# xuelunshen/gim

Hardware: AMD Instinct MI355X
Metric: image-pairs/sec at 640x480 (higher is better)
Workload: dtype fp16

## Files before the change

### gim_amd/csrc/emit.hip

```cpp
#include "gim_common.h"

namespace {

struct Segs { gim_copy_segs s; };

__global__ void __launch_bounds__(256) copy_segments_kernel(const Segs a) {
    const int k = blockIdx.y;
    const char* src = (const char*)a.s.src[k];
    char* dst = (char*)a.s.dst[k];
    const int64_t n = a.s.bytes[k];
    const int64_t t = (int64_t)blockIdx.x * blockDim.x + threadIdx.x, nt = (int64_t)gridDim.x * blockDim.x;
    const bool vec = (((uintptr_t)src | (uintptr_t)dst) & 15) == 0;
    const int64_t nv = vec ? n >> 4 : 0;
    for (int64_t i = t; i < nv; i += nt) ((uint4*)dst)[i] = src ? ((const uint4*)src)[i] : make_uint4(0u, 0u, 0u, 0u);
    for (int64_t i = (nv << 4) + t; i < n; i += nt) dst[i] = src ? src[i] : (char)0;
}

__global__ void __launch_bounds__(256) pack_matches_kernel(const int64_t* __restrict__ m_bids, const float2* __restrict__ mk0,
                                                           const float2* __restrict__ mk1, const float* __restrict__ conf,
                                                           const int64_t* __restrict__ pair_ids, int64_t pid_base,
                                                           float* __restrict__ out, int M) {
    const int m = blockIdx.x * blockDim.x + threadIdx.x;
    if (m >= M) return;
    const int64_t b = m_bids[m];
    const float pid = (float)(pair_ids ? pair_ids[b] : pid_base + b);
    const float2 p0 = mk0[m], p1 = mk1[m];
    float* o = out + (size_t)m * 6;
    *(float2*)(o + 0) = make_float2(pid, p0.x);
    *(float2*)(o + 2) = make_float2(p0.y, p1.x);
    *(float2*)(o + 4) = make_float2(p1.y, conf[m]);
}

constexpr int TL_THREADS = 1024, TL_MAX_FLAGS = 32768;

template <bool REACH2, bool QUARTER>
__device__ __forceinline__ void fine_tile_list_body(const int64_t* __restrict__ b_ids, const int64_t* __restrict__ i_ids,
                                                    const int64_t* __restrict__ j_ids, const int* __restrict__ count, int cap,
                                                    int bs, int w0c, int w1c, int stride, int H, int W,
                                                    int* __restrict__ tiles, int* __restrict__ n_tiles, int tiles_cap,
                                                    int* __restrict__ tiles2, int* __restrict__ n_tiles2,
                                                    int* __restrict__ tilesq, int* __restrict__ n_tilesq, int tilesq_cap) {
    static_assert(!QUARTER || REACH2, "the quarter-level lists are derived from the +-4 flags");
    __shared__ __attribute__((aligned(16))) unsigned char flags[TL_MAX_FLAGS];
    __shared__ int part[TL_THREADS];
    __shared__ int part2[REACH2 ? TL_THREADS : 1];
    __shared__ int partq[QUARTER ? TL_THREADS : 1][2];
    const int t = threadIdx.x;
    const int tiles_x = (W + 31) / 32, tiles_y = (H + 7) / 8, per_img = tiles_x * tiles_y, nflags = 2 * bs * per_img;
    const int h = H / 2, w = W / 2, qtiles_x = w / 32, qtiles_y = h / 8, qper_img = qtiles_x * qtiles_y;
    const int qbase = (nflags + 3) & ~3, nqflags = QUARTER ? 2 * bs * qper_img : 0;
    for (int i = t; i < (QUARTER ? qbase + nqflags : nflags); i += TL_THREADS) flags[i] = 0;
    __syncthreads();
    int M = count[0];
    M = M < 0 ? 0 : (M < cap ? M : cap);
    for (int m = t; m < M; m += TL_THREADS) {
        const int64_t b = b_ids[m];
        if (b < 0 || b >= bs) continue;
#pragma unroll
        for (int side = 0; side < 2; ++side) {
            const int64_t cell = side ? j_ids[m] : i_ids[m];
            const int wc = side ? w1c : w0c;
            if (cell < 0 || cell >= (int64_t)wc * ((H + stride - 1) / stride)) continue;
            const int cy = (int)cell / wc, cx = (int)cell - cy * wc;
            int y0 = cy * stride - 3, y1 = cy * stride + 3, x0 = cx * stride - 3, x1 = cx * stride + 3;
            y0 = y0 < 0 ? 0 : y0; x0 = x0 < 0 ? 0 : x0;
            y1 = y1 > H - 1 ? H - 1 : y1; x1 = x1 > W - 1 ? W - 1 : x1;
            if (y0 > y1 || x0 > x1) continue;
            const int img = side * bs + (int)b;
            if constexpr (REACH2) {
                int Y0 = cy * stride - 4, Y1 = cy * stride + 4, X0 = cx * stride - 4, X1 = cx * stride + 4;
                Y0 = Y0 < 0 ? 0 : Y0; X0 = X0 < 0 ? 0 : X0;
                Y1 = Y1 > H - 1 ? H - 1 : Y1; X1 = X1 > W - 1 ? W - 1 : X1;
                for (int ty = Y0 >> 3; ty <= (Y1 >> 3); ++ty)
                    for (int tx = X0 >> 5; tx <= (X1 >> 5); ++tx) {
                        const bool in3 = ty >= (y0 >> 3) && ty <= (y1 >> 3) && tx >= (x0 >> 5) && tx <= (x1 >> 5);
                        const int f = (img * tiles_y + ty) * tiles_x + tx;
                        atomicOr((unsigned*)flags + (f >> 2), (in3 ? 3u : 2u) << (8 * (f & 3)));
                    }
            } else {
            for (int ty = y0 >> 3; ty <= (y1 >> 3); ++ty)
                for (int tx = x0 >> 5; tx <= (x1 >> 5); ++tx) flags[(img * tiles_y + ty) * tiles_x + tx] = 1;
            }
        }
    }
    __syncthreads();
    if constexpr (QUARTER) {
        unsigned char* const qf = flags + qbase;
        const float sy = (float)(h - 1) / (float)(H - 1), sx = (float)(w - 1) / (float)(W - 1);
        for (int i = t; i < nflags; i += TL_THREADS) {
            if (!(flags[i] & 2)) continue;
            const int img = i / per_img, r = i - img * per_img, ty = r / tiles_x, tx = r - ty * tiles_x;
            const int xa = (int)(sx * (32 * tx));
            const int xe = xa + 23 < w - 1 ? xa + 23 : w - 1;
            for (int Y = 8 * ty; Y < 8 * ty + 8 && Y < H; ++Y) {
                const float fy = sy * Y;
                const int y0 = (int)fy, y1 = y0 + (y0 < h - 1 ? 1 : 0);
#pragma unroll
                for (int d = 0; d < 3; ++d) {
                    const int ra = y0 - d > 0 ? y0 - d : 0, rb = y1 + d < h - 1 ? y1 + d : h - 1;
                    const int ca = xa - d > 0 ? xa - d : 0, cb = xe + d < w - 1 ? xe + d : w - 1;
                    const unsigned bits = d == 0 ? 7u : (d == 1 ? 6u : 4u);
                    for (int qy = ra >> 3; qy <= (rb >> 3); ++qy)
                        for (int qx = ca >> 5; qx <= (cb >> 5); ++qx) {
                            const int f = (img * qtiles_y + qy) * qtiles_x + qx;
                            if ((qf[f] & bits) != bits) atomicOr((unsigned*)qf + (f >> 2), bits << (8 * (f & 3)));
                        }
                }
            }
        }
        __syncthreads();
    }
    const int per = (nflags + TL_THREADS - 1) / TL_THREADS;
    const int lo = t * per < nflags ? t * per : nflags, hi = lo + per < nflags ? lo + per : nflags;
    int n = 0, n2 = 0;
    for (int i = lo; i < hi; ++i) { n += flags[i] & 1; n2 += flags[i] >> 1; }
    part[t] = n;
    if constexpr (REACH2) part2[t] = n2;
    const int qper = (nqflags + TL_THREADS - 1) / TL_THREADS;
    const int qlo = t * qper < nqflags ? t * qper : nqflags, qhi = qlo + qper < nqflags ? qlo + qper : nqflags;
    int nab = 0, nc = 0;
    if constexpr (QUARTER) {
        for (int i = qlo; i < qhi; ++i) {
            const int f = flags[qbase + i];
            nab += ((f >> 2) & 1) << 16 | ((f >> 1) & 1);
            nc += f & 1;
        }
        partq[t][0] = nab; partq[t][1] = nc;
    }
    __syncthreads();
    for (int d = 1; d < TL_THREADS; d <<= 1) {
        const int v = t >= d ? part[t - d] : 0;
        const int v2 = REACH2 && t >= d ? part2[t - d] : 0;
        const int vab = QUARTER && t >= d ? partq[t - d][0] : 0, vc = QUARTER && t >= d ? partq[t - d][1] : 0;
        __syncthreads();
        part[t] += v;
        if constexpr (REACH2) part2[t] += v2;
        if constexpr (QUARTER) { partq[t][0] += vab; partq[t][1] += vc; }
        __syncthreads();
    }
    int o = part[t] - n;
    for (int i = lo; i < hi; ++i)
        if (flags[i] & 1) {
            if (o < tiles_cap) tiles[o] = i;
            ++o;
        }
    if (t == TL_THREADS - 1) n_tiles[0] = part[t] < tiles_cap ? part[t] : tiles_cap;
    if constexpr (REACH2) {
        int o2 = part2[t] - n2;
        for (int i = lo; i < hi; ++i)
            if (flags[i] & 2) {
                if (o2 < tiles_cap) tiles2[o2] = i;
                ++o2;
            }
        if (t == TL_THREADS - 1) n_tiles2[0] = part2[t] < tiles_cap ? part2[t] : tiles_cap;
    }
    if constexpr (QUARTER) {
        int oa = (partq[t][0] >> 16) - (nab >> 16), ob = (partq[t][0] & 0xffff) - (nab & 0xffff), oc = partq[t][1] - nc;
        for (int i = qlo; i < qhi; ++i) {
            const int f = flags[qbase + i];
            if (f & 4) { if (oa < tilesq_cap) tilesq[oa] = i; ++oa; }
            if (f & 2) { if (ob < tilesq_cap) tilesq[tilesq_cap + ob] = i; ++ob; }
            if (f & 1) { if (oc < tilesq_cap) tilesq[2 * tilesq_cap + oc] = i; ++oc; }
        }
        if (t == TL_THREADS - 1) {
            const int ta = partq[t][0] >> 16, tb = partq[t][0] & 0xffff, tc = partq[t][1];
            n_tilesq[0] = ta < tilesq_cap ? ta : tilesq_cap;
            n_tilesq[1] = tb < tilesq_cap ? tb : tilesq_cap;
            n_tilesq[2] = tc < tilesq_cap ? tc : tilesq_cap;
        }
    }
}

template <bool REACH2>
__global__ void __launch_bounds__(TL_THREADS) fine_tile_list_kernel(const int64_t* __restrict__ b_ids, const int64_t* __restrict__ i_ids,
                                                                  const int64_t* __restrict__ j_ids, const int* __restrict__ count, int cap,
                                                                  int bs, int w0c, int w1c, int stride, int H, int W,
                                                                  int* __restrict__ tiles, int* __restrict__ n_tiles, int tiles_cap,
                                                                  int* __restrict__ tiles2, int* __restrict__ n_tiles2) {
    fine_tile_list_body<REACH2, false>(b_ids, i_ids, j_ids, count, cap, bs, w0c, w1c, stride, H, W, tiles, n_tiles, tiles_cap, tiles2, n_tiles2,
                                       nullptr, nullptr, 0);
}

__global__ void __launch_bounds__(TL_THREADS) fine_tile_lists4_kernel(const int64_t* __restrict__ b_ids, const int64_t* __restrict__ i_ids,
                                                                    const int64_t* __restrict__ j_ids, const int* __restrict__ count, int cap,
                                                                    int bs, int w0c, int w1c, int stride, int H, int W,
                                                                    int* __restrict__ tiles, int* __restrict__ n_tiles, int tiles_cap,
                                                                    int* __restrict__ tiles2, int* __restrict__ n_tiles2,
                                                                    int* __restrict__ tilesq, int* __restrict__ n_tilesq, int tilesq_cap) {
    fine_tile_list_body<true, true>(b_ids, i_ids, j_ids, count, cap, bs, w0c, w1c, stride, H, W, tiles, n_tiles, tiles_cap, tiles2, n_tiles2,
                                    tilesq, n_tilesq, tilesq_cap);
}

}

extern "C" int gim_fine_tile_list_max_flags(void) { return TL_MAX_FLAGS; }

extern "C" int gim_fine_tile_list(const int64_t* b_ids, const int64_t* i_ids, const int64_t* j_ids, const int* count, int cap, int bs,
                                  int w0c, int w1c, int stride, int H, int W, int* tiles, int* n_tiles, int tiles_cap, gim_stream_t stream) {
    GIM_REQUIRE(b_ids && i_ids && j_ids && count && tiles && n_tiles, "gim_fine_tile_list: NULL pointer");
    GIM_REQUIRE(cap >= 0 && bs > 0 && w0c > 0 && w1c > 0 && stride > 0 && H > 0 && W > 0, "gim_fine_tile_list: bad geometry");
    const int64_t nflags = 2ll * bs * ((W + 31) / 32) * ((H + 7) / 8);
    GIM_REQUIRE(nflags <= TL_MAX_FLAGS, "gim_fine_tile_list: %lld patches exceed the %d flags of the one-workgroup kernel", (long long)nflags, TL_MAX_FLAGS);
    GIM_REQUIRE(tiles_cap >= nflags, "gim_fine_tile_list: the list holds %d entries, the maps have %lld patches", tiles_cap, (long long)nflags);
    hipLaunchKernelGGL(fine_tile_list_kernel<false>, dim3(1), dim3(TL_THREADS), 0, (hipStream_t)stream, b_ids, i_ids, j_ids, count, cap, bs, w0c, w1c,
                       stride, H, W, tiles, n_tiles, tiles_cap, nullptr, nullptr);
    return gim_check_launch("fine_tile_list_kernel");
}

extern "C" int gim_fine_tile_lists(const int64_t* b_ids, const int64_t* i_ids, const int64_t* j_ids, const int* count, int cap, int bs,
                                   int w0c, int w1c, int stride, int H, int W, int* tiles, int* n_tiles, int* tiles4, int* n_tiles4,
                                   int tiles_cap, gim_stream_t stream) {
    GIM_REQUIRE(b_ids && i_ids && j_ids && count && tiles && n_tiles && tiles4 && n_tiles4, "gim_fine_tile_lists: NULL pointer");
    GIM_REQUIRE(cap >= 0 && bs > 0 && w0c > 0 && w1c > 0 && stride > 0 && H > 0 && W > 0, "gim_fine_tile_lists: bad geometry");
    const int64_t nflags = 2ll * bs * ((W + 31) / 32) * ((H + 7) / 8);
    GIM_REQUIRE(nflags <= TL_MAX_FLAGS, "gim_fine_tile_lists: %lld patches exceed the %d flags of the one-workgroup kernel", (long long)nflags, TL_MAX_FLAGS);
    GIM_REQUIRE(tiles_cap >= nflags, "gim_fine_tile_lists: the lists hold %d entries each, the maps have %lld patches", tiles_cap, (long long)nflags);
    hipLaunchKernelGGL(fine_tile_list_kernel<true>, dim3(1), dim3(TL_THREADS), 0, (hipStream_t)stream, b_ids, i_ids, j_ids, count, cap, bs, w0c, w1c,
                       stride, H, W, tiles, n_tiles, tiles_cap, tiles4, n_tiles4);
    return gim_check_launch("fine_tile_list_kernel");
}

extern "C" int gim_fine_tile_lists4(const int64_t* b_ids, const int64_t* i_ids, const int64_t* j_ids, const int* count, int cap, int bs,
                                    int w0c, int w1c, int stride, int H, int W, int* tiles, int* n_tiles, int* tiles4, int* n_tiles4,
                                    int tiles_cap, int* tilesq, int* n_tilesq, int tilesq_cap, gim_stream_t stream) {
    GIM_REQUIRE(b_ids && i_ids && j_ids && count && tiles && n_tiles && tiles4 && n_tiles4 && tilesq && n_tilesq, "gim_fine_tile_lists4: NULL pointer");
    GIM_REQUIRE(cap >= 0 && bs > 0 && w0c > 0 && w1c > 0 && stride > 0 && H > 0 && W > 0, "gim_fine_tile_lists4: bad geometry");
    GIM_REQUIRE(H % 16 == 0 && W % 64 == 0, "gim_fine_tile_lists4: the 1/4-resolution maps (%d x %d) must be whole 8 x 32 patches", H / 2, W / 2);
    const int64_t nflags = 2ll * bs * (W / 32) * (H / 8), nq = 2ll * bs * (W / 64) * (H / 16);
    GIM_REQUIRE(((nflags + 3) & ~3ll) + nq <= TL_MAX_FLAGS, "gim_fine_tile_lists4: %lld + %lld patches exceed the %d flags of the one-workgroup kernel",
                (long long)nflags, (long long)nq, TL_MAX_FLAGS);
    GIM_REQUIRE(tiles_cap >= nflags && tilesq_cap >= nq, "gim_fine_tile_lists4: the lists hold %d / %d entries each, the maps have %lld / %lld patches",
                tiles_cap, tilesq_cap, (long long)nflags, (long long)nq);
    hipLaunchKernelGGL(fine_tile_lists4_kernel, dim3(1), dim3(TL_THREADS), 0, (hipStream_t)stream, b_ids, i_ids, j_ids, count, cap, bs, w0c, w1c,
                       stride, H, W, tiles, n_tiles, tiles_cap, tiles4, n_tiles4, tilesq, n_tilesq, tilesq_cap);
    return gim_check_launch("fine_tile_lists4_kernel");
}

extern "C" int gim_copy_segments(const gim_copy_segs* sp, gim_stream_t stream) {
    GIM_REQUIRE(sp, "gim_copy_segments: NULL args");
    GIM_REQUIRE(sp->n >= 0 && sp->n <= GIM_MAX_COPY_SEGS, "gim_copy_segments: n=%d outside [0, %d]", sp->n, GIM_MAX_COPY_SEGS);
    int64_t mx = 0;
    for (int k = 0; k < sp->n; ++k) {
        GIM_REQUIRE(sp->bytes[k] >= 0 && (sp->bytes[k] == 0 || sp->dst[k]), "gim_copy_segments: segment %d: bad size / NULL dst", k);
        mx = sp->bytes[k] > mx ? sp->bytes[k] : mx;
    }
    if (sp->n == 0 || mx == 0) return GIM_OK;
    Segs a;
    a.s = *sp;
    int64_t blocks = (mx / 16 + 255) / 256;
    blocks = blocks < 1 ? 1 : (blocks > 1024 ? 1024 : blocks);
    hipLaunchKernelGGL(copy_segments_kernel, dim3((unsigned)blocks, (unsigned)sp->n), dim3(256), 0, (hipStream_t)stream, a);
    return gim_check_launch("copy_segments_kernel");
}

extern "C" int gim_pack_matches(const int64_t* m_bids, const float* mkpts0, const float* mkpts1, const float* mconf,
                                const int64_t* pair_ids, int64_t pid_base, float* out, int M, gim_stream_t stream) {
    GIM_REQUIRE(M >= 0, "gim_pack_matches: M=%d", M);
    if (M == 0) return GIM_OK;
    GIM_REQUIRE(m_bids && mkpts0 && mkpts1 && mconf && out, "gim_pack_matches: NULL pointer");
    hipLaunchKernelGGL(pack_matches_kernel, dim3((unsigned)((M + 255) / 256)), dim3(256), 0, (hipStream_t)stream, m_bids,
                       (const float2*)mkpts0, (const float2*)mkpts1, mconf, pair_ids, pid_base, out, M);
    return gim_check_launch("pack_matches_kernel");
}
```

Before: 970.8.

## Rewrite four-list tile kernel with wave-shuffle scans, prefetch and word-wide popcounts

```diff
diff --git a/gim_amd/csrc/emit.hip b/gim_amd/csrc/emit.hip
--- a/gim_amd/csrc/emit.hip
+++ b/gim_amd/csrc/emit.hip
@@ -33,23 +33,18 @@
 
 constexpr int TL_THREADS = 1024, TL_MAX_FLAGS = 32768;
 
-template <bool REACH2, bool QUARTER>
+template <bool REACH2>
 __device__ __forceinline__ void fine_tile_list_body(const int64_t* __restrict__ b_ids, const int64_t* __restrict__ i_ids,
                                                     const int64_t* __restrict__ j_ids, const int* __restrict__ count, int cap,
                                                     int bs, int w0c, int w1c, int stride, int H, int W,
                                                     int* __restrict__ tiles, int* __restrict__ n_tiles, int tiles_cap,
-                                                    int* __restrict__ tiles2, int* __restrict__ n_tiles2,
-                                                    int* __restrict__ tilesq, int* __restrict__ n_tilesq, int tilesq_cap) {
-    static_assert(!QUARTER || REACH2, "the quarter-level lists are derived from the +-4 flags");
+                                                    int* __restrict__ tiles2, int* __restrict__ n_tiles2) {
     __shared__ __attribute__((aligned(16))) unsigned char flags[TL_MAX_FLAGS];
     __shared__ int part[TL_THREADS];
     __shared__ int part2[REACH2 ? TL_THREADS : 1];
-    __shared__ int partq[QUARTER ? TL_THREADS : 1][2];
     const int t = threadIdx.x;
     const int tiles_x = (W + 31) / 32, tiles_y = (H + 7) / 8, per_img = tiles_x * tiles_y, nflags = 2 * bs * per_img;
-    const int h = H / 2, w = W / 2, qtiles_x = w / 32, qtiles_y = h / 8, qper_img = qtiles_x * qtiles_y;
-    const int qbase = (nflags + 3) & ~3, nqflags = QUARTER ? 2 * bs * qper_img : 0;
-    for (int i = t; i < (QUARTER ? qbase + nqflags : nflags); i += TL_THREADS) flags[i] = 0;
+    for (int i = t; i < nflags; i += TL_THREADS) flags[i] = 0;
     __syncthreads();
     int M = count[0];
     M = M < 0 ? 0 : (M < cap ? M : cap);
@@ -84,58 +79,19 @@
         }
     }
     __syncthreads();
-    if constexpr (QUARTER) {
-        unsigned char* const qf = flags + qbase;
-        const float sy = (float)(h - 1) / (float)(H - 1), sx = (float)(w - 1) / (float)(W - 1);
-        for (int i = t; i < nflags; i += TL_THREADS) {
-            if (!(flags[i] & 2)) continue;
-            const int img = i / per_img, r = i - img * per_img, ty = r / tiles_x, tx = r - ty * tiles_x;
-            const int xa = (int)(sx * (32 * tx));
-            const int xe = xa + 23 < w - 1 ? xa + 23 : w - 1;
-            for (int Y = 8 * ty; Y < 8 * ty + 8 && Y < H; ++Y) {
-                const float fy = sy * Y;
-                const int y0 = (int)fy, y1 = y0 + (y0 < h - 1 ? 1 : 0);
-#pragma unroll
-                for (int d = 0; d < 3; ++d) {
-                    const int ra = y0 - d > 0 ? y0 - d : 0, rb = y1 + d < h - 1 ? y1 + d : h - 1;
-                    const int ca = xa - d > 0 ? xa - d : 0, cb = xe + d < w - 1 ? xe + d : w - 1;
-                    const unsigned bits = d == 0 ? 7u : (d == 1 ? 6u : 4u);
-                    for (int qy = ra >> 3; qy <= (rb >> 3); ++qy)
-                        for (int qx = ca >> 5; qx <= (cb >> 5); ++qx) {
-                            const int f = (img * qtiles_y + qy) * qtiles_x + qx;
-                            if ((qf[f] & bits) != bits) atomicOr((unsigned*)qf + (f >> 2), bits << (8 * (f & 3)));
-                        }
-                }
-            }
-        }
-        __syncthreads();
-    }
     const int per = (nflags + TL_THREADS - 1) / TL_THREADS;
     const int lo = t * per < nflags ? t * per : nflags, hi = lo + per < nflags ? lo + per : nflags;
     int n = 0, n2 = 0;
     for (int i = lo; i < hi; ++i) { n += flags[i] & 1; n2 += flags[i] >> 1; }
     part[t] = n;
     if constexpr (REACH2) part2[t] = n2;
-    const int qper = (nqflags + TL_THREADS - 1) / TL_THREADS;
-    const int qlo = t * qper < nqflags ? t * qper : nqflags, qhi = qlo + qper < nqflags ? qlo + qper : nqflags;
-    int nab = 0, nc = 0;
-    if constexpr (QUARTER) {
-        for (int i = qlo; i < qhi; ++i) {
-            const int f = flags[qbase + i];
-            nab += ((f >> 2) & 1) << 16 | ((f >> 1) & 1);
-            nc += f & 1;
-        }
-        partq[t][0] = nab; partq[t][1] = nc;
-    }
     __syncthreads();
     for (int d = 1; d < TL_THREADS; d <<= 1) {
         const int v = t >= d ? part[t - d] : 0;
         const int v2 = REACH2 && t >= d ? part2[t - d] : 0;
-        const int vab = QUARTER && t >= d ? partq[t - d][0] : 0, vc = QUARTER && t >= d ? partq[t - d][1] : 0;
         __syncthreads();
         part[t] += v;
         if constexpr (REACH2) part2[t] += v2;
-        if constexpr (QUARTER) { partq[t][0] += vab; partq[t][1] += vc; }
         __syncthreads();
     }
     int o = part[t] - n;
@@ -154,20 +110,167 @@
             }
         if (t == TL_THREADS - 1) n_tiles2[0] = part2[t] < tiles_cap ? part2[t] : tiles_cap;
     }
-    if constexpr (QUARTER) {
-        int oa = (partq[t][0] >> 16) - (nab >> 16), ob = (partq[t][0] & 0xffff) - (nab & 0xffff), oc = partq[t][1] - nc;
-        for (int i = qlo; i < qhi; ++i) {
-            const int f = flags[qbase + i];
-            if (f & 4) { if (oa < tilesq_cap) tilesq[oa] = i; ++oa; }
-            if (f & 2) { if (ob < tilesq_cap) tilesq[tilesq_cap + ob] = i; ++ob; }
-            if (f & 1) { if (oc < tilesq_cap) tilesq[2 * tilesq_cap + oc] = i; ++oc; }
-        }
-        if (t == TL_THREADS - 1) {
-            const int ta = partq[t][0] >> 16, tb = partq[t][0] & 0xffff, tc = partq[t][1];
-            n_tilesq[0] = ta < tilesq_cap ? ta : tilesq_cap;
-            n_tilesq[1] = tb < tilesq_cap ? tb : tilesq_cap;
-            n_tilesq[2] = tc < tilesq_cap ? tc : tilesq_cap;
-        }
+}
+
+constexpr int TL_WAVES = TL_THREADS / 64, TL_AHEAD = 3;
+
+template <int width>
+__device__ __forceinline__ unsigned tl_wave_scan(unsigned v, int lane) {
+#pragma unroll
+    for (int d = 1; d < width; d <<= 1) {
+        const unsigned u = __shfl_up(v, d);
+        if (lane >= d) v += u;
+    }
+    return v;
+}
+
+__device__ __forceinline__ void tl_or(unsigned* word, unsigned bits) {
+    if ((__hip_atomic_load(word, __ATOMIC_RELAXED, __HIP_MEMORY_SCOPE_WORKGROUP) & bits) != bits) atomicOr(word, bits);
+}
+
+__device__ __forceinline__ void fine_tile_lists4_body(const int64_t* __restrict__ b_ids, const int64_t* __restrict__ i_ids,
+                                                      const int64_t* __restrict__ j_ids, const int* __restrict__ count, int cap,
+                                                      int bs, int w0c, int w1c, int stride, int H, int W,
+                                                      int* __restrict__ tiles, int* __restrict__ n_tiles, int tiles_cap,
+                                                      int* __restrict__ tiles2, int* __restrict__ n_tiles2,
+                                                      int* __restrict__ tilesq, int* __restrict__ n_tilesq, int tilesq_cap) {
+    __shared__ uint4 flags16[TL_MAX_FLAGS / 16];
+    __shared__ unsigned wsum[TL_WAVES][3];
+    const unsigned char* const flags = (const unsigned char*)flags16;
+    unsigned* const fw = (unsigned*)flags16;
+    const int t = threadIdx.x, lane = t & 63, wave = t >> 6;
+    const int tiles_x = W / 32, tiles_y = H / 8, per_img = tiles_x * tiles_y, nflags = 2 * bs * per_img;
+    const int h = H / 2, w = W / 2, qtiles_x = w / 32, qtiles_y = h / 8, qper_img = qtiles_x * qtiles_y;
+    const int qbase = (nflags + 3) & ~3, nqflags = 2 * bs * qper_img;
+
+    int64_t nb[TL_AHEAD], ni[TL_AHEAD], nj[TL_AHEAD];
+    auto fetch = [&](int m0) {
+#pragma unroll
+        for (int k = 0; k < TL_AHEAD; ++k) {
+            const int m = m0 + k * TL_THREADS < cap ? m0 + k * TL_THREADS : cap - 1;
+            nb[k] = b_ids[m]; ni[k] = i_ids[m]; nj[k] = j_ids[m];
+        }
+    };
+    if (cap > 0) fetch(t);
+    int M = count[0];
+    M = M < 0 ? 0 : (M < cap ? M : cap);
+    for (int i = t; i < (qbase + nqflags + 15) / 16; i += TL_THREADS) flags16[i] = make_uint4(0u, 0u, 0u, 0u);
+    __syncthreads();
+
+    const int rows_c = (H + stride - 1) / stride;
+    for (int m0 = t; m0 < M; m0 += TL_AHEAD * TL_THREADS) {
+        int b[TL_AHEAD], c[TL_AHEAD][2];
+#pragma unroll
+        for (int k = 0; k < TL_AHEAD; ++k) {
+            const bool live = m0 + k * TL_THREADS < M;
+            b[k] = !live || nb[k] < 0 || nb[k] >= bs ? -1 : (int)nb[k];
+            c[k][0] = ni[k] < 0 || ni[k] >= (int64_t)w0c * rows_c ? -1 : (int)ni[k];
+            c[k][1] = nj[k] < 0 || nj[k] >= (int64_t)w1c * rows_c ? -1 : (int)nj[k];
+        }
+        if (m0 + TL_AHEAD * TL_THREADS < M) fetch(m0 + TL_AHEAD * TL_THREADS);
+#pragma unroll
+        for (int k = 0; k < TL_AHEAD; ++k) {
+            if (b[k] < 0) continue;
+#pragma unroll
+            for (int side = 0; side < 2; ++side) {
+                const int cell = c[k][side], wc = side ? w1c : w0c;
+                if (cell < 0) continue;
+                const int cy = cell / wc, cx = cell - cy * wc;
+                int y0 = cy * stride - 3, y1 = cy * stride + 3, x0 = cx * stride - 3, x1 = cx * stride + 3;
+                y0 = y0 < 0 ? 0 : y0; x0 = x0 < 0 ? 0 : x0;
+                y1 = y1 > H - 1 ? H - 1 : y1; x1 = x1 > W - 1 ? W - 1 : x1;
+                if (y0 > y1 || x0 > x1) continue;
+                const int img = side * bs + b[k];
+                int Y0 = cy * stride - 4, Y1 = cy * stride + 4, X0 = cx * stride - 4, X1 = cx * stride + 4;
+                Y0 = Y0 < 0 ? 0 : Y0; X0 = X0 < 0 ? 0 : X0;
+                Y1 = Y1 > H - 1 ? H - 1 : Y1; X1 = X1 > W - 1 ? W - 1 : X1;
+                for (int ty = Y0 >> 3; ty <= (Y1 >> 3); ++ty)
+                    for (int tx = X0 >> 5; tx <= (X1 >> 5); ++tx) {
+                        const bool in3 = ty >= (y0 >> 3) && ty <= (y1 >> 3) && tx >= (x0 >> 5) && tx <= (x1 >> 5);
+                        const int f = (img * tiles_y + ty) * tiles_x + tx;
+                        tl_or(fw + (f >> 2), (in3 ? 3u : 2u) << (8 * (f & 3)));
+                    }
+            }
+        }
+    }
+    __syncthreads();
+
+    {
+        const float sy = (float)(h - 1) / (float)(H - 1), sx = (float)(w - 1) / (float)(W - 1);
+        for (int i = t; i < nflags; i += TL_THREADS) {
+            if (!(flags[i] & 2)) continue;
+            const int img = i / per_img, r = i - img * per_img, ty = r / tiles_x, tx = r - ty * tiles_x;
+            const int xa = (int)(sx * (32 * tx));
+            const int xe = xa + 23 < w - 1 ? xa + 23 : w - 1;
+            const float fy = sy * (8 * ty), fl = sy * (8 * ty + 7);
+            const int y0 = (int)fy, yl = (int)fl, y1 = yl + (yl < h - 1 ? 1 : 0);
+            int ra[3], rb[3], ca[3], cb[3];
+#pragma unroll
+            for (int d = 0; d < 3; ++d) {
+                ra[d] = (y0 - d > 0 ? y0 - d : 0) >> 3; rb[d] = (y1 + d < h - 1 ? y1 + d : h - 1) >> 3;
+                ca[d] = (xa - d > 0 ? xa - d : 0) >> 5; cb[d] = (xe + d < w - 1 ? xe + d : w - 1) >> 5;
+            }
+            for (int qy = ra[2]; qy <= rb[2]; ++qy)
+                for (int qx = ca[2]; qx <= cb[2]; ++qx) {
+                    const bool in1 = qy >= ra[1] && qy <= rb[1] && qx >= ca[1] && qx <= cb[1];
+                    const bool in0 = qy >= ra[0] && qy <= rb[0] && qx >= ca[0] && qx <= cb[0];
+                    const int f = qbase + (img * qtiles_y + qy) * qtiles_x + qx;
+                    tl_or(fw + (f >> 2), (in0 ? 7u : (in1 ? 6u : 4u)) << (8 * (f & 3)));
+                }
+        }
+    }
+    __syncthreads();
+
+    const int per = (nflags + 4 * TL_THREADS - 1) / (4 * TL_THREADS) * 4, qper = (nqflags + 4 * TL_THREADS - 1) / (4 * TL_THREADS) * 4;
+    const int lo = t * per < nflags ? t * per : nflags, hi = lo + per < nflags ? lo + per : nflags;
+    const int qlo = t * qper < nqflags ? t * qper : nqflags, qhi = qlo + qper < nqflags ? qlo + qper : nqflags;
+    unsigned n34 = 0, nab = 0, nc = 0;
+    for (int i = lo; i < hi; i += 4) {
+        const unsigned v = fw[i >> 2];
+        n34 += __popc(v & 0x01010101u) + (__popc(v & 0x02020202u) << 16);
+    }
+    for (int i = qlo; i < qhi; i += 4) {
+        const unsigned v = fw[(qbase + i) >> 2];
+        nab += __popc(v & 0x02020202u) + (__popc(v & 0x04040404u) << 16);
+        nc += __popc(v & 0x01010101u);
+    }
+    const unsigned s34 = tl_wave_scan<64>(n34, lane), sab = tl_wave_scan<64>(nab, lane), sc = tl_wave_scan<64>(nc, lane);
+    if (lane == 63) { wsum[wave][0] = s34; wsum[wave][1] = sab; wsum[wave][2] = sc; }
+    __syncthreads();
+    const unsigned w34 = tl_wave_scan<TL_WAVES>(lane < TL_WAVES ? wsum[lane][0] : 0u, lane);
+    const unsigned wab = tl_wave_scan<TL_WAVES>(lane < TL_WAVES ? wsum[lane][1] : 0u, lane);
+    const unsigned wc = tl_wave_scan<TL_WAVES>(lane < TL_WAVES ? wsum[lane][2] : 0u, lane);
+    const int before = wave ? wave - 1 : 0;
+    const unsigned o34 = (wave ? __shfl(w34, before) : 0u) + s34 - n34, oab = (wave ? __shfl(wab, before) : 0u) + sab - nab;
+    int o = (int)(o34 & 0xffffu), o2 = (int)(o34 >> 16);
+    for (int i = lo; i < hi; i += 4) {
+        const unsigned v = fw[i >> 2];
+#pragma unroll
+        for (int k = 0; k < 4; ++k) {
+            const unsigned f = v >> (8 * k);
+            if (f & 1u) { if (o < tiles_cap) tiles[o] = i + k; ++o; }
+            if (f & 2u) { if (o2 < tiles_cap) tiles2[o2] = i + k; ++o2; }
+        }
+    }
+    int oa = (int)(oab >> 16), ob = (int)(oab & 0xffffu), oc = (int)((wave ? __shfl(wc, before) : 0u) + sc - nc);
+    for (int i = qlo; i < qhi; i += 4) {
+        const unsigned v = fw[(qbase + i) >> 2];
+#pragma unroll
+        for (int k = 0; k < 4; ++k) {
+            const unsigned f = v >> (8 * k);
+            if (f & 4u) { if (oa < tilesq_cap) tilesq[oa] = i + k; ++oa; }
+            if (f & 2u) { if (ob < tilesq_cap) tilesq[tilesq_cap + ob] = i + k; ++ob; }
+            if (f & 1u) { if (oc < tilesq_cap) tilesq[2 * tilesq_cap + oc] = i + k; ++oc; }
+        }
+    }
+    const unsigned t34 = __shfl(w34, TL_WAVES - 1), tab = __shfl(wab, TL_WAVES - 1), tc = __shfl(wc, TL_WAVES - 1);
+    if (t == 0) {
+        const int n3 = (int)(t34 & 0xffffu), n4 = (int)(t34 >> 16), ta = (int)(tab >> 16), tb = (int)(tab & 0xffffu);
+        n_tiles[0] = n3 < tiles_cap ? n3 : tiles_cap;
+        n_tiles2[0] = n4 < tiles_cap ? n4 : tiles_cap;
+        n_tilesq[0] = ta < tilesq_cap ? ta : tilesq_cap;
+        n_tilesq[1] = tb < tilesq_cap ? tb : tilesq_cap;
+        n_tilesq[2] = (int)tc < tilesq_cap ? (int)tc : tilesq_cap;
     }
 }
 
@@ -177,8 +280,7 @@
                                                                   int bs, int w0c, int w1c, int stride, int H, int W,
                                                                   int* __restrict__ tiles, int* __restrict__ n_tiles, int tiles_cap,
                                                                   int* __restrict__ tiles2, int* __restrict__ n_tiles2) {
-    fine_tile_list_body<REACH2, false>(b_ids, i_ids, j_ids, count, cap, bs, w0c, w1c, stride, H, W, tiles, n_tiles, tiles_cap, tiles2, n_tiles2,
-                                       nullptr, nullptr, 0);
+    fine_tile_list_body<REACH2>(b_ids, i_ids, j_ids, count, cap, bs, w0c, w1c, stride, H, W, tiles, n_tiles, tiles_cap, tiles2, n_tiles2);
 }
 
 __global__ void __launch_bounds__(TL_THREADS) fine_tile_lists4_kernel(const int64_t* __restrict__ b_ids, const int64_t* __restrict__ i_ids,
@@ -187,8 +289,8 @@
                                                                     int* __restrict__ tiles, int* __restrict__ n_tiles, int tiles_cap,
                                                                     int* __restrict__ tiles2, int* __restrict__ n_tiles2,
                                                                     int* __restrict__ tilesq, int* __restrict__ n_tilesq, int tilesq_cap) {
-    fine_tile_list_body<true, true>(b_ids, i_ids, j_ids, count, cap, bs, w0c, w1c, stride, H, W, tiles, n_tiles, tiles_cap, tiles2, n_tiles2,
-                                    tilesq, n_tilesq, tilesq_cap);
+    fine_tile_lists4_body(b_ids, i_ids, j_ids, count, cap, bs, w0c, w1c, stride, H, W, tiles, n_tiles, tiles_cap, tiles2, n_tiles2, tilesq, n_tilesq,
+                          tilesq_cap);
 }
 
 }
```

Measured after the change: 979.3 (median of 6 runs). No clear change (+0.9%).
